# xandergos/terrain-diffusion

Measured on AMD Instinct MI355X. Metric: terrain megapixels/sec (decoded) at fixed steps, 30m model, higher is better.
Workload: dtype bf16; 1 GPU; BASELINE configs[2]: terrain-diffusion-30m base U-Net, 8x8 tile grid (stride 32, 288x288 latents) with overlap blending, 20 steps, 64 windows batched per solver step; edm_steps=20, parallelism=1 independent streams (one process per GPU, no data-path collective)

## Files before the change

### terrain_diffusion_amd/csrc/conv_fewcout.hip

```cpp
#include "conv_common.h"

namespace td {

template <typename T> __device__ __forceinline__ float fewcout_dot2(unsigned a, unsigned b, float c);
template <> __device__ __forceinline__ float fewcout_dot2<__bf16>(unsigned a, unsigned b, float c) {
    typedef __bf16 bx2 __attribute__((ext_vector_type(2)));
    return __builtin_amdgcn_fdot2_f32_bf16(__builtin_bit_cast(bx2, a), __builtin_bit_cast(bx2, b), c, false);
}
template <> __device__ __forceinline__ float fewcout_dot2<_Float16>(unsigned a, unsigned b, float c) {
    typedef _Float16 hx2 __attribute__((ext_vector_type(2)));
    return __builtin_amdgcn_fdot2(__builtin_bit_cast(hx2, a), __builtin_bit_cast(hx2, b), c, false);
}

template <typename T, int CO>
__global__ __launch_bounds__(256) void conv_fewcout_kernel(const ConvParams p) {
    constexpr int TW = 16, TH = 16, PW = 18, NPATCH = PW * PW, PITCH = 144, CHUNK = 64;
    constexpr int W_BASE = NPATCH * PITCH;
    extern __shared__ __attribute__((aligned(16))) unsigned char smem[];
    const int tid = threadIdx.x;
    unsigned b = blockIdx.x;
    const int txi = (int)(b % (unsigned)p.tiles_x); b /= (unsigned)p.tiles_x;
    const int tyi = (int)(b % (unsigned)p.tiles_y); const int n0 = (int)(b / (unsigned)p.tiles_y);
    const int y0 = tyi * TH, x0 = txi * TW;
    const ConvSeg& sg = p.seg[0];
// ... 34 lines not shown
                const u32x4 xv = *(const u32x4*)(xp + q * 16);
#pragma unroll
                for (int c = 0; c < CO; ++c) {
                    const u32x4 wv = *(const u32x4*)(smem + W_BASE + ((tap * CO + c) * 8 + q) * 16);
                    float a = acc[c][q >> 2];
#pragma unroll
                    for (int i = 0; i < 4; ++i) a = fewcout_dot2<T>(xv[i], wv[i], a);
                    acc[c][q >> 2] = a;
                }
            }
        }
    }
    const int y = y0 + ly, x = x0 + lx;
    if (y < H && x < W) {
        if (p.epi == EPI_DPM_STEP) {
            f32x4 v = {0.f, 0.f, 0.f, 0.f};
#pragma unroll
            for (int c = 0; c < CO; ++c) v[c] = acc[c][0] + acc[c][1];
            (void)epilogue4<T>(p, n0, y, x, 0, v, 0.f, v);
            return;
        }
        float* o = (float*)p.out + (size_t)((n0 * H + y) * W + x) * p.out_cstride;
#pragma unroll
        for (int c = 0; c < CO; ++c) if (c < p.Cout) o[c] = acc[c][0] + acc[c][1];
    }
}

template <typename T, int CO>
static hipError_t launch_fewcout_cfg(const ConvParams& p, hipStream_t st) {
    constexpr size_t LDS = (size_t)18 * 18 * 144 + (size_t)9 * CO * 128;
    const long long grid = (long long)p.tiles_x * p.tiles_y * p.N;
    if (grid <= 0 || grid >= ((long long)1 << 31)) return hipErrorInvalidValue;
    hipLaunchKernelGGL((conv_fewcout_kernel<T, CO>), dim3((unsigned)grid), dim3(256), LDS, st, p);
    return hipGetLastError();
}

hipError_t launch_conv_fewcout(const ConvParams& p, int dtype, hipStream_t st) {
    if (p.nseg != 1 || p.seg[0].taps != 9 || p.seg[0].xform != 0 || p.seg[0].resample != 0 || p.seg[0].Hs != p.H || p.seg[0].Ws != p.W || (p.seg[0].C & 63) || p.seg[0].C < 64)
        return hipErrorInvalidValue;
    if (p.epi == EPI_DPM_STEP && (!p.dpm_x || !p.dpm_m1 || !p.dpm_xin || p.dpm_xin_cstride < p.Cout || (p.dpm_k.order == 3 && !p.dpm_m2))) return hipErrorInvalidValue;
    if ((p.epi != EPI_PLAIN && p.epi != EPI_DPM_STEP) || !p.out_f32 || p.ksplit != 1 || p.res || p.out2 || p.out_sumsq || p.clip > 0.f || p.Cout < 1 || p.Cout > 4 || p.out_cstride < p.Cout)
        return hipErrorInvalidValue;
    if (p.tiles_x != (p.W + 15) / 16 || p.tiles_y != (p.H + 15) / 16) return hipErrorInvalidValue;
    const int co = p.Cout <= 1 ? 1 : p.Cout <= 2 ? 2 : 4;
    if (dtype == 2) return co == 1 ? launch_fewcout_cfg<_Float16, 1>(p, st) : co == 2 ? launch_fewcout_cfg<_Float16, 2>(p, st) : launch_fewcout_cfg<_Float16, 4>(p, st);
    return co == 1 ? launch_fewcout_cfg<__bf16, 1>(p, st) : co == 2 ? launch_fewcout_cfg<__bf16, 2>(p, st) : launch_fewcout_cfg<__bf16, 4>(p, st);
}

}
```

### terrain_diffusion_amd/csrc/conv_glds_wide.hip

```cpp
#include "conv_common.h"

namespace td {

#ifdef TD_TRACE
#define TDW_T(v) unsigned long long v = __builtin_amdgcn_s_memtime(); asm volatile("s_waitcnt lgkmcnt(0)" ::: "memory")
#define TDW_TACC(acc, a, b) acc += (b) - (a)
#else
#define TDW_T(v)
#define TDW_TACC(acc, a, b)
#endif

template <typename T, int BN, bool TAIL, bool PERS>
__global__ __launch_bounds__(256, 2) void conv_glds_kernel_wide(const ConvParams p) {
    static_assert(!(TAIL && PERS), "the persistent tile loop serves pure 3x3 launches");
    typedef typename Half<T>::x8 hx8;
    constexpr int NTHR = 256, TH = 16, TW = 16, TPIX = 256;
    constexpr int PW = 18, NPATCH = 18 * 18;
    constexpr int WM = 64, MT = 2, NT = BN / 32;
    constexpr int CHUNK = 64, HALF = 32, PER16 = 8;
    constexpr int WNT = PERS ? 128 : NTHR, PNT = PERS ? 128 : NTHR;
    constexpr int A_ITERS = (NPATCH * 4 + PNT - 1) / PNT;
    constexpr int A_FULL = NPATCH * 4 / PNT, A_REM = NPATCH * 4 - A_FULL * PNT;
    constexpr int NBI = (BN * 64 + WNT * 16 - 1) / (WNT * 16), PSTR = WNT * 16;
    constexpr int H_BYTES = BN * 64, RING = 4;
    constexpr bool HAS_DUMP = (BN * 64) % (WNT * 16) != 0;
    constexpr int DUMP_BASE = RING * H_BYTES;
    constexpr int PITCH = 80;
    constexpr int A_BASE = DUMP_BASE + (HAS_DUMP ? 2048 : 0), A_BYTES = NPATCH * PITCH;
    constexpr int RN_BASE = A_BASE + 2 * A_BYTES, RN_BYTES = (NPATCH * 4 + 15) / 16 * 16;
// ... 126 lines not shown
#define TDW_STORE_A(BUF, RNP) TDW_STORE_R(BUF, RNP, 0, A_ITERS)
#define TDW_STORE_R(BUF, RNP, I0, I1)                                                                  \
    {                                                                                                  \
        _Pragma("unroll") for (int it_ = (I0); it_ < (I1); ++it_) {                                    \
            if (it_ < A_FULL || pt < A_REM) {                                                          \
                u32x4 v_ = aoff[it_] >= 0 ? av[it_] : u32x4{0u, 0u, 0u, 0u};                           \
                if (seg_xform != 0 && aoff[it_] >= 0) {                                \
                    float s_ = seg_scale;                                                              \
                    if (seg_xform == 2) s_ *= (RNP)[(pt >> 2) + it_ * (PNT / 4)];                      \
                    v_ = xform_piece<T>(v_, s_);                                                       \
                }                                                                                      \
                *(u32x4*)(smem + st_base + ((BUF) * A_BYTES + it_ * (PNT / 4) * PITCH)) = v_;          \
            }                                                                                          \
        }                                                                                              \
    }
    const bool r_want = !TAIL && k_epi == EPI_RESIDUAL && k_hres;
    bool r_pref = false;
    const T* r_ptr[MT];
#define TDW_R_ADDR()                                                                                                  \
    {                                                                                                                 \
        TDW_FRESH()                                                                                                   \
        const int rHs_ = KA(res_Hs), rWs_ = KA(res_Ws), rrs_ = KA(res_resample), rcs_ = KA(res_cstride);              \
        _Pragma("unroll") for (int i_ = 0; i_ < MT; ++i_) {                                                           \
            int img_, ty_, tx_;                                                                                       \
            frag_pixel<TW, TPIX>(wm * WM + i_ * 32, l31, img_, ty_, tx_);                                             \
            const int y_ = y0 + ty_, x_ = x0 + tx_;                                                                   \
            const int sp_ = (n0 < k_N && y_ < k_H && x_ < k_W) ? src_pixel(n0, y_, x_, rHs_, rWs_, rrs_) : 0;         \
            r_ptr[i_] = (const T*)KA(res) + (sp_ * rcs_ + co0 + 8 * lh);                                              \
        }                                                                                                             \
    }
#define TDW_R_UNIT(Q) (*(const u32x4*)(r_ptr[(Q) / NU] + ((co0 + (((Q) % NU) >> 1) * 32 < k_Cout) ? (((Q) % NU) >> 1) * 32 + ((Q) & 1) * 16 : 0)))
// ... 62 lines not shown
#define TDW_FRAG_READ(WF, XF, SLOT, KS, BUF, TOFF)                                                           \
    {                                                                                                        \
        _Pragma("unroll") for (int j_ = 0; j_ < NT; ++j_) WF[j_] = *(const u32x4*)(smem + (wbase[KS] + (SLOT)) + j_ * 2048);    \
        _Pragma("unroll") for (int i_ = 0; i_ < MT; ++i_) XF[i_] = *(const u32x4*)(smem + xbase[i_] + ((BUF) * A_BYTES + (TOFF) + (KS) * 32)); \
    }
#define TDW_FRAG_MFMA(WF, XF)                                                                                \
    {                                                                                                        \
        _Pragma("unroll") for (int i_ = 0; i_ < MT; ++i_)                                                    \
            _Pragma("unroll") for (int j_ = 0; j_ < NT; ++j_)                                                \
                acc[i_][j_] = Half<T>::mfma32(__builtin_bit_cast(hx8, WF[j_]), __builtin_bit_cast(hx8, XF[i_]), acc[i_][j_]); \
    }
#define TDW_HS(S)                                                                                            \
    {                                                                                                        \
        TDW_T(tA_);                                                                                          \
         \
        if ((S) == 1 || (S) == 2 || (((S) == 10 || (S) == 11) && nxt)) asm volatile("s_waitcnt vmcnt(%0)" ::"n"(A_ITERS + NBI) : "memory"); \
        else if ((S) >= 16 && !nxt) { if (r_now) asm volatile("s_waitcnt vmcnt(%0)" ::"n"(A_ITERS) : "memory"); else asm volatile("s_waitcnt vmcnt(0)" ::: "memory"); } \
        else asm volatile("s_waitcnt vmcnt(%0)" ::"n"(NBI) : "memory");                                      \
        if ((S) == 6 || (S) == 15) asm volatile("s_waitcnt lgkmcnt(0)" ::: "memory");    \
        TDW_T(tM_); TDW_TACC(tr_stage, tA_, tM_);    \
        __builtin_amdgcn_s_barrier();                                                                        \
        asm volatile("" ::: "memory");                                                                       \
        TDW_T(tB_); TDW_TACC(tr_wait, tA_, tB_);                                                             \
        if ((S) == 3 || ((S) == 12 && nxt)) TDW_PIN_A()    \
        if ((S) + 3 < 18 || nxt) TDW_DMA((S) + 3);    \
        if ((S) == 0) TDW_LOAD_A(chunk, 1);                                                                  \
        if ((S) == 9 && nxt) { if (newseg) TDW_SEG_BEGIN(seg + 1); TDW_LOAD_A(newseg ? 0 : chunk + 1, 0); }  \
        if ((S) == 15 && r_now) TDW_LOAD_R()                                                                 \
        if ((S) == 5) TDW_STORE_A(1, s_rn);                                                                        \
        if ((S) == 14 && nxt) TDW_STORE_A(0, s_rn);                                                                \
        TDW_FRAG_MFMA(wfA_, xfA_);                                                                           \
        if ((S) < 17 || nxt) TDW_FRAG_READ(wfA_, xfA_, rslot, 0, (((S) + 1) / 9) & 1, TDW_TOFF(((S) + 1) % 9)); \
        TDW_FRAG_MFMA(wfB_, xfB_);                                                                           \
        if ((S) < 17 || nxt) { TDW_FRAG_READ(wfB_, xfB_, rslot, 1, (((S) + 1) / 9) & 1, TDW_TOFF(((S) + 1) % 9)); TDW_SLOT_NEXT(rslot) } \
        __builtin_amdgcn_sched_group_barrier(0x008, MT * NT, 0);                                             \
        __builtin_amdgcn_sched_group_barrier(0x100, NT + MT, 0);                                             \
        __builtin_amdgcn_sched_group_barrier(0x008, MT * NT, 0);                                             \
        __builtin_amdgcn_sched_group_barrier(0x100, NT + MT, 0);                                             \
    }
#define TDW_B0 4
#define TDW_B1 8
#define TDW_HSP(S)                                                                                           \
    {                                                                                                        \
        if (w_role) {                                                                                        \
            if ((S) >= 16 && !nxt) asm volatile("s_waitcnt vmcnt(0)" ::: "memory");                          \
            else if (((S) == 10 || (S) == 11) && nxt) asm volatile("s_waitcnt vmcnt(%0)" ::"n"(NBI + 1) : "memory"); \
            else asm volatile("s_waitcnt vmcnt(%0)" ::"n"(NBI) : "memory");                                  \
        } else {                                                                                             \
            if ((S) == 5 || ((S) == 14 && nxt)) asm volatile("s_waitcnt vmcnt(%0)" ::"n"(A_ITERS - TDW_B0) : "memory"); \
// ... 52 lines not shown
        asm volatile("" ::: "memory");
        TDW_FRAG_READ(wfA_, xfA_, rslot, 0, 0, TDW_TOFF(0));
        TDW_FRAG_READ(wfB_, xfB_, rslot, 1, 0, TDW_TOFF(0));
        TDW_SLOT_NEXT(rslot)
    }
    const bool no_tail = n3 == p.kgroups;
#ifdef TD_TRACE
    unsigned long long tr_loop = 0;
#endif
    for (;;) {
    const bool has_next = PERS && vb + vstep < k_grid;
    if (n3 > 0) {
        for (int u = 0; u < n3; ++u) {
            const bool last = u + 1 == n3;
            const bool wrap = PERS && last && has_next;
            const bool nxt = !last || wrap;
            const bool newseg = !last && chunk + 1 == seg_nchunks;
            const bool r_now = r_want && last && no_tail;
            if constexpr (PERS) {
                TDW_HSP(0); TDW_HSP(1); TDW_HSP(2); TDW_HSP(3); TDW_HSP(4); TDW_HSP(5); TDW_HSP(6); TDW_HSP(7); TDW_HSP(8);
                TDW_HSP(9); TDW_HSP(10); TDW_HSP(11); TDW_HSP(12); TDW_HSP(13); TDW_HSP(14); TDW_HSP(15); TDW_HSP(16); TDW_HSP(17);
            } else {
                TDW_HS(0); TDW_HS(1); TDW_HS(2); TDW_HS(3); TDW_HS(4); TDW_HS(5); TDW_HS(6); TDW_HS(7); TDW_HS(8);
                TDW_HS(9); TDW_HS(10); TDW_HS(11); TDW_HS(12); TDW_HS(13); TDW_HS(14); TDW_HS(15); TDW_HS(16); TDW_HS(17);
            }
            if (wrap) { seg = 0; chunk = 0; } else if (newseg) { ++seg; chunk = 0; } else ++chunk;
        }
    }
    if constexpr (TAIL) {
    if (n3 < p.kgroups && p.dma1x1) {
        constexpr int STAGE = TPIX * 64, NSTG = 3;
        static_assert(NSTG * STAGE <= 2 * A_BYTES, "stage buffers over the two halo patches");
        int pseg = n3 > 0 ? seg + 1 : 0, pchunk = 0, phf = 0, pn = 1;
        const T* psrc = nullptr;
        unsigned poff[4];
#define TDW_P_BEGIN()                                                                                                 \
// ... 225 lines not shown
#ifdef TD_TRACE
    TDW_T(tr_eissue);
    asm volatile("s_waitcnt vmcnt(0)" ::: "memory");
    TDW_T(tr_end);
    if (lane == 0) {
        unsigned long long* tb = (unsigned long long*)p.partial + ((size_t)blockIdx.x * 4 + wave) * 16;
        tb[0] = tr_pro - tr_start; tb[1] = tr_loop - tr_pro; tb[2] = tr_end - tr_loop; tb[3] = tr_wait; tb[4] = tr_stage; tb[5] = tr_start; tb[6] = tr_end;
        tb[8] = tr_rt0; tb[9] = ((unsigned long long)__builtin_amdgcn_s_getreg((31 << 11) | 4) << 8) | __builtin_amdgcn_s_getreg((3 << 11) | 20);
        tb[10] = __builtin_amdgcn_s_memrealtime();
        tb[7] = tb[10] - tr_rt0; tb[11] = tr_end - tr_eissue;
    }
#endif
#undef TDW_R_ADDR
#undef TDW_R_UNIT
#undef TDW_LOAD_R
}

template <typename T, int BN, bool TAIL, bool PERS>
static hipError_t launch_glds_wide_cfg2(const ConvParams& p, hipStream_t st) {
    constexpr int NPATCH = 18 * 18;
    constexpr size_t RING_BYTES = 4 * (size_t)(BN * 64) + ((BN * 64) % 4096 ? 2048 : 0);
    constexpr size_t LDS = RING_BYTES + 2 * (size_t)NPATCH * 80 + (PERS ? 2 : 1) * ((size_t)(NPATCH * 4 + 15) / 16 * 16 + (PERS ? (size_t)512 : (size_t)BN * 4));
    static_assert(2 * LDS <= 160 * 1024, "two workgroups per CU");
    if (p.ksplit != 1 || p.W < 16 || p.CoutPad % BN || p.nseg < 1 || p.nseg > 3) return hipErrorInvalidValue;
    if (p.out_f32 || (p.Cout & 7) || p.epi == EPI_DPM_STEP) return hipErrorInvalidValue;
    bool seen1 = false;
    for (int s = 0; s < p.nseg; ++s) { if (p.seg[s].taps == 9 && seen1) return hipErrorInvalidValue; if (p.seg[s].taps != 9) seen1 = true; }
    ConvParams pd = p;
    for (int s = p.nseg; s < 3; ++s) { pd.seg[s].C = 0; pd.seg[s].taps = 0; }
    pd.dma1x1 = 1;
    for (int s = 0; s < p.nseg; ++s) if (p.seg[s].taps != 9 && p.seg[s].xform != 0) pd.dma1x1 = 0;
    const int mtiles = p.tiles_x * p.tiles_y * p.img_groups, grid = p.n_ntiles * mtiles;
    if (grid <= 0 || (long long)grid * std::max(mtiles, p.n_ntiles) >= ((long long)1 << 32)) return hipErrorInvalidValue;
    pd.sb_d0 = mtiles; pd.sb_m0 = td_magic(mtiles); pd.sb_d1 = p.n_ntiles; pd.sb_m1 = td_magic(p.n_ntiles); pd.sb_m2 = td_magic(p.tiles_x); pd.sb_m3 = td_magic(p.tiles_y);
    pd.sb_grid = grid; pd.sb_grid8 = (grid & 7) == 0 ? (unsigned)grid >> 3 : 0u;
    int launch_grid = grid;
    if (PERS) {
        if (p.persist <= 0 || p.persist > grid || (p.H & 15) || (p.W & 15) || p.Cout != p.CoutPad || p.kgroups < 1) return hipErrorInvalidValue;
        if (pd.sb_grid8 && (p.persist & 7)) return hipErrorInvalidValue;
        launch_grid = p.persist;
    }
    auto kern = conv_glds_kernel_wide<T, BN, TAIL, PERS>;
    static bool attr_set[64] = {};
    int dev_ = 0; (void)hipGetDevice(&dev_);
    if (dev_ < 0 || dev_ >= 64 || !attr_set[dev_]) {
        hipError_t e = hipFuncSetAttribute((const void*)kern, hipFuncAttributeMaxDynamicSharedMemorySize, (int)LDS);
        if (e != hipSuccess) return e;
        if (dev_ >= 0 && dev_ < 64) attr_set[dev_] = true;
    }
    hipLaunchKernelGGL(kern, dim3(launch_grid), dim3(256), LDS, st, pd);
    return hipGetLastError();
}

inline int conv_wide_persist_grid(long long tiles, int slots) {
    if (tiles < 2LL * slots) return 0;
    const long long rounds = (tiles + slots - 1) / slots;
    long long g = (tiles + rounds - 1) / rounds;
    if ((tiles & 7) == 0) g = (g + 7) & ~7LL;
    return (int)std::min<long long>(g, tiles);
}

template <typename T, int BN>
static hipError_t launch_glds_wide_cfg(const ConvParams& p, hipStream_t st) {
    bool tail = false;
    for (int s = 0; s < p.nseg; ++s) if (p.seg[s].taps != 9) tail = true;
    if (p.persist > 0) {
        if constexpr (BN == 64) return tail ? hipErrorInvalidValue : launch_glds_wide_cfg2<T, BN, false, true>(p, st);
        else return hipErrorInvalidValue;
    }
    return tail ? launch_glds_wide_cfg2<T, BN, true, false>(p, st) : launch_glds_wide_cfg2<T, BN, false, false>(p, st);
}

hipError_t launch_conv_glds_wide(const ConvParams& p, int dtype, int bn, hipStream_t st) {
    if (dtype == 2) {
        if (bn == 96) return launch_glds_wide_cfg<_Float16, 96>(p, st);
        if (bn == 64) return launch_glds_wide_cfg<_Float16, 64>(p, st);
        return hipErrorInvalidValue;
    }
    if (bn == 96) return launch_glds_wide_cfg<__bf16, 96>(p, st);
    if (bn == 64) return launch_glds_wide_cfg<__bf16, 64>(p, st);
    return hipErrorInvalidValue;
}

}
```

### terrain_diffusion_amd/csrc/engine.hip

```cpp
#include <hip/hip_runtime.h>
#include <math.h>
#include <stdio.h>
#include <string.h>

#include <map>
#include <memory>
#include <string>
#include <vector>
#include <unordered_map>

#include "../../include/td_engine.h"
#include "td_device.h"

#include "conv_igemm.hip"
#include "conv_glds.hip"
#include "conv_glds_wide.hip"
#include "conv_sb.hip"
#include "conv_s16.hip"
#include "conv_fewcout.hip"
#include "small_kernels.hip"
#include "compose_kernels.hip"
#include "attn_mfma.hip"

using namespace td;
// ... 589 lines not shown
static int new_buf(Plan& pl, size_t bytes, void** out) {
    Buf b(new DevBuf());
    HIP_TRY(b->alloc(bytes, true));
    *out = b->p;
    pl.bytes += b->bytes;
    pl.bufs.push_back(std::move(b));
    return TD_OK;
}

struct SegSpec { const Tensor* t; int C; int taps; int resample; int xform; float scale; };

static int build_plan(td_unet* u, int N, int H, int W, Plan** out, int lane = 0) {
    static const char* const kPlanOptions[] = {"batch_invariant", "glds", "splitk", "producer_act", "glds_min_wgs", "glds_variant", "glds_bn",
                                               "glds_splitk", "glds_splitk_max", "glds_splitk_min_groups", "splitk_target_wgs",
                                               "bn128_min_wgs", "attn_mfma", "glds_splitk_from_groups", "glds_bn64", "glds_small_max_groups", "glds_round_aware", "walk_alternate", "glds_tiny", "glds_dma1x1", "splitk_weighted",
                                               "sb", "sb_target_wgs", "sb_mt", "sb_nt", "sb_order", "sb_max_glds_wgs", "sb_splitk", "sb_splitk_wgs", "sb_splitk_max", "s16", "s16_min_wgs", "sb_m4", "glds_wide", "glds_wide_min_wgs", "glds_wide_tail", "glds_wide_persist", "fewcout"};
    std::string key = std::to_string(N) + "_" + std::to_string(H) + "_" + std::to_string(W);
    for (const char* o : kPlanOptions) key += "_" + std::to_string((long long)u->eng->option(o, -7));
    if (lane) key += "_lane" + std::to_string(lane);
    auto it = u->plans.find(key);
    if (it != u->plans.end()) { it->second->last_use = ++u->use_clock; *out = it->second.get(); return TD_OK; }
    if (N < 1 || N > 1023 || H > 1023 || W > 1023) return fail(TD_ERR_ARG, "batch/size out of range");
    const int down = 1 << (u->cfg.n_levels - 1);
    if (H % down || W % down) return fail(TD_ERR_ARG, "H and W must be divisible by 2^(levels-1)");
    {
        const size_t budget = (size_t)u->eng->option("plan_cache_mb", 65536) << 20;
        const size_t max_plans = (size_t)u->eng->option("plan_cache_max", 12);
        size_t total = 0;
        for (auto& kv : u->plans) total += kv.second->bytes;
        while (!u->plans.empty() && (total > budget || u->plans.size() >= max_plans)) {
            auto victim = u->plans.begin();
// ... 36 lines not shown
        memset(&p, 0, sizeof p);
        p.nseg = (int)segs.size();
        int kgroups = 0;
        for (int i = 0; i < p.nseg; ++i) {
            const SegSpec& s = segs[i];
            ConvSeg& d = p.seg[i];
            d.src = s.t->ptr; d.C = (s.C + chunk - 1) / chunk * chunk; d.cstride = s.t->cstride; d.Hs = s.t->H; d.Ws = s.t->W;
            if ((size_t)N * d.Hs * d.Ws * (size_t)d.cstride >= ((size_t)1 << 31))
                return fail(TD_ERR_ARG, "batch too large for 32-bit activation addressing (N*H*W*C >= 2^31 elements in " + label + "): split the batch");
            d.taps = s.taps; d.resample = s.resample; d.xform = s.xform; d.scale = s.scale;
            if (s.xform == 2) {
                if (!s.t->sumsq) return fail(TD_ERR_STATE, "pixel-norm source without sumsq: " + label);
                d.sumsq = s.t->sumsq; d.nparts = s.t->nparts; d.inv_c = 1.f / (float)s.t->C;
            }
            kgroups += d.C / chunk;
            op.k_alg += (double)cw.segs[i].c_real * s.taps;
            if (cw.segs[i].c_pad != d.C || cw.segs[i].taps != d.taps) return fail(TD_ERR_STATE, "segment/weight mismatch: " + label);
        }
        p.wpack = cw.packed->p;
        p.N = N; p.H = h; p.W = w; p.Cout = cw.cout; p.CoutPad = cw.cout_pad; p.kgroups = kgroups;
        op.narrow = w < 16;
        {
            const int TW2 = op.narrow ? 8 : 16;
            const bool c128 = cw.cout_pad % 128 == 0, c96 = cw.cout_pad % 96 == 0;
            auto tiles = [&](int TH, int NIMG) { return (int64_t)((w + TW2 - 1) / TW2) * ((h + TH - 1) / TH) * ((N + NIMG - 1) / NIMG); };
            const bool c64 = !op.narrow && u->eng->option("glds_bn64", 1) != 0;
            auto pick_bn = [&](int64_t mt) { return (c128 && (mt * (cw.cout_pad / 128) >= 512 || !c96)) ? 128 : (c96 ? 96 : (c64 ? 64 : 0)); };
            const int64_t mt_big = tiles(op.narrow ? 8 : 16, op.narrow ? 4 : 1), mt_small = tiles(8, op.narrow ? 2 : 1);
            int variant = 0, bn2 = pick_bn(mt_big);
            if (bn2 && mt_big * (cw.cout_pad / bn2) < 1024) { variant = 1; bn2 = pick_bn(mt_small); }
// ... 32 lines not shown
                {
                    const int64_t wmode = u->eng->option("glds_wide", 1);
                    const int bnw = cw.cout_pad % 96 == 0 ? 96 : (cw.cout_pad % 64 == 0 ? 64 : 0);
                    const int64_t tmode = u->eng->option("glds_wide_tail", 1);
                    bool pure3 = true;
                    for (const SegSpec& sg : segs) if (sg.taps != 9 && (sg.xform != 0 || tmode == 0 || (tmode == 1 && bnw != 64))) pure3 = false;
                    const int64_t wgs_w = bnw ? tiles(16, 1) * (cw.cout_pad / bnw) : 0;
                    if (wmode != 0 && !inv && fv < 0 && fbn == 0 && !op.narrow && p.ksplit == 1 && bnw && !out_f32 && (cw.cout & 7) == 0 && p.nseg <= 3 && (pure3 || wmode == 2) &&
                        (wmode == 2 || wgs_w >= u->eng->option("glds_wide_min_wgs", 384))) {
                        op.glds_variant = 3; op.bn = bnw;
                        p.tiles_x = (w + 15) / 16; p.tiles_y = (h + 15) / 16; p.img_groups = N; p.n_ntiles = cw.cout_pad / bnw;
                        bool tail3 = false;
                        for (const SegSpec& sg : segs) if (sg.taps != 9) tail3 = true;
                        if (u->eng->option("glds_wide_persist", 0) != 0 && bnw == 64 && !tail3 && (h & 15) == 0 && (w & 15) == 0 && cw.cout == cw.cout_pad)
                            p.persist = conv_wide_persist_grid((long long)p.tiles_x * p.tiles_y * N * p.n_ntiles, 2 * std::max(1, u->eng->n_cus));
                    }
                }
                if (op.flavor == 2 && sb_takes && op.glds_variant != 3) {
                    {
                        const int TWs = op.narrow ? 8 : 16;
                        auto th_of = [&](int mt) { return op.narrow ? (mt == 2 ? 8 : 4) : (mt == 4 ? 8 : mt == 2 ? 4 : 2); };
                        auto sb_wgs = [&](int mt, int nt) { return (int64_t)((w + TWs - 1) / TWs) * ((h + th_of(mt) - 1) / th_of(mt)) * N * (cw.cout_pad / (32 * nt)); };
                        const int64_t target = u->eng->option("sb_target_wgs", 160);
                        int mt = 1, nt = 1, ks = 1;
                        if (!op.narrow && u->eng->option("sb_m4", 0) != 0 && sb_wgs(2, 2) >= target && sb_wgs(4, 1) >= target) { mt = 4; nt = 1; }
                        else if (sb_wgs(2, 2) >= target) { mt = 2; nt = 2; } else if (sb_wgs(2, 1) >= target) { mt = 2; nt = 1; }
                        else if (use_splitk && u->eng->option("sb_splitk", 1) != 0 && sb_wgs(2, 1) * 2 <= u->eng->option("sb_splitk_wgs", 224)) {
                            mt = 2; nt = 1;
                            ks = (int)std::min<int64_t>(std::min<int64_t>(kgroups, u->eng->option("sb_splitk_max", 16)), (u->eng->option("sb_splitk_wgs", 224) + sb_wgs(2, 1) / 2) / sb_wgs(2, 1));
                        }
// ... 30 lines not shown
            }
        }
        if (op.flavor == 0) {
            const int TH = 8, TW = op.narrow ? 8 : 16, NIMG = op.narrow ? 2 : 1;
            p.tiles_x = (w + TW - 1) / TW; p.tiles_y = (h + TH - 1) / TH; p.img_groups = (N + NIMG - 1) / NIMG;
            const int64_t mt = (int64_t)p.tiles_x * p.tiles_y * p.img_groups;
            op.bn = 64;
            const bool inv0 = u->eng->option("batch_invariant", 0) != 0;
            if (cw.cout_pad % 128 == 0 && (inv0 || mt * (cw.cout_pad / 128) >= bn128_min)) op.bn = 128;
            else if (cw.cout_pad % 96 == 0 && (inv0 || mt * (cw.cout_pad / 96) >= bn128_min)) op.bn = 96;
            p.n_ntiles = cw.cout_pad / op.bn;
            const int64_t base = mt * p.n_ntiles;
            p.ksplit = 1;
            if (use_splitk && !u->eng->option("batch_invariant", 0) && base < splitk_target / 2 && kgroups > 1) p.ksplit = (int)std::min<int64_t>(kgroups, (splitk_target + base - 1) / base);
        }
        if (u->eng->option("fewcout", 1) != 0 && (u->dt == 1 || u->dt == 2) && out_f32 && epi == EPI_PLAIN && cw.cout <= 4 && segs.size() == 1 && segs[0].taps == 9 &&
            segs[0].xform == 0 && p.seg[0].resample == 0 && p.seg[0].Hs == h && p.seg[0].Ws == w && !res && clip <= 0.f && (int64_t)h * w >= 128 * 128 && w >= 16) {
            op.flavor = 6; op.bn = 64; op.glds_variant = 0; op.narrow = false;
            p.tiles_x = (w + 15) / 16; p.tiles_y = (h + 15) / 16; p.img_groups = N; p.n_ntiles = 1; p.ksplit = 1; p.persist = 0;
        }
        if (p.ksplit > 64) p.ksplit = 64;
        if (!conv_set_kbounds(p, u->eng->option("splitk_weighted", 1) != 0, chunk)) return fail(TD_ERR_UNSUPPORTED, "split-K bounds: " + label);
        p.epi = epi; p.out_f32 = out_f32 ? 1 : 0; p.clip = clip; p.zeros = u->eng->zeros;
        const int out_parts = p.ksplit > 1 ? (cw.cout_pad + 255) / 256 : op.flavor == 5 ? cw.cout_pad / 16 : (op.flavor >= 2 ? cw.cout_pad / 32 : p.n_ntiles * 2);
        if (out_f32) {
            outT->C = cw.cout; outT->cstride = 8; outT->H = h; outT->W = w; outT->sumsq = nullptr;
            if ((rc = new_buf(pl, (size_t)N * h * w * 8 * 4, &outT->ptr))) return rc;
        } else if ((rc = new_tensor(cw.cout, h, w, want_sumsq, out_parts, outT))) return rc;
        p.out = outT->ptr; p.out_cstride = outT->cstride; p.out_sumsq = outT->sumsq;
        if ((size_t)N * h * w * (size_t)std::max(outT->cstride, cw.cout_pad) >= ((size_t)1 << 31))
            return fail(TD_ERR_ARG, "batch too large for 32-bit activation addressing (output of " + label + "): split the batch");
        op.cvec_off = cvec_off; p.cvec_stride = u->c_total;
        if (res) {
            p.res = res->ptr; p.res_cstride = res->cstride; p.res_Hs = res->H; p.res_Ws = res->W; p.res_resample = res_resample;
// ... 237 lines not shown
        }
        mark();
        hipError_t e = op.flavor == 6 ? launch_conv_fewcout(p, u->dt, st)
                       : op.flavor == 5 ? launch_conv_s16(p, u->dt, op.narrow, st)
                       : op.flavor == 4 ? launch_conv_sb(p, u->dt, op.narrow, op.sb_mt, op.sb_nt, st)
                       : op.flavor == 2 ? (op.glds_variant == 3 ? launch_conv_glds_wide(p, u->dt, op.bn, st) : launch_conv_glds(p, u->dt, op.narrow, op.bn, op.glds_variant, st))
                       : launch_conv(p, u->dt, op.narrow, op.bn, 0, st);
        mark(); if (prof) { ev_kind.push_back(0); char tag[160]; double gf_ = op.k_alg * 2.0 * p.N * p.H * p.W * p.Cout * 1e-9;
            double mb_ = 0.0; const double es_ = (double)u->esize();
            for (int si_ = 0; si_ < p.nseg; ++si_) mb_ += (double)p.N * p.seg[si_].Hs * p.seg[si_].Ws * p.seg[si_].C * es_ + (double)p.seg[si_].C / 64.0 * p.seg[si_].taps * p.CoutPad * 128.0 * (es_ / 2.0);
            if (p.res) mb_ += (double)p.N * p.res_Hs * p.res_Ws * p.Cout * es_;
            const double o1_ = (double)p.N * p.H * p.W * p.Cout * (p.out_f32 ? 4.0 : es_);
            const double mbs_ = (mb_ + o1_) * 1e-6;
            mb_ += o1_ * (p.out2 ? 2.0 : 1.0);
            mb_ *= 1e-6;
            snprintf(tag, sizeof tag, " [%dx%d k%d f%d%s bn%d wg%d ks%d gf%.2f mb%.2f mbs%.2f]", p.H, p.W, p.kgroups, op.flavor, op.flavor == 5 ? "c16" : op.flavor == 4 ? (op.sb_mt == 4 ? "m4n1" : op.sb_mt == 2 ? (op.sb_nt == 2 ? "m2n2" : "m2n1") : (op.sb_nt == 2 ? "m1n2" : "m1n1")) : op.flavor == 2 ? (op.glds_variant == 3 ? (p.persist > 0 ? "wp" : "w") : op.glds_variant == 2 ? "t" : op.glds_variant ? "s" : "b") : "", op.bn, p.n_ntiles * p.tiles_x * p.tiles_y * p.img_groups, p.ksplit, gf_, mb_, mbs_); ev_label.push_back(op.label + tag);
            ev_flop.push_back(op.flavor == 2 ? 2.0 * p.N * p.H * p.W * (double)p.Cout * op.k_alg : 0.0); }
        if (e != hipSuccess) return fail(TD_ERR_HIP, "conv launch " + op.label + ": " + hipGetErrorString(e));
    }
    return TD_OK;
}

static inline dim3 grid1(size_t n, int b = 256) { return dim3((unsigned)((n + b - 1) / b)); }

extern "C" {

const char* td_last_error(void) { return g_err.c_str(); }
int td_version(void) { return 1; }
#ifndef TD_CSRC_SHA
#define TD_CSRC_SHA "unstamped"
#endif
// ... 34 lines not shown
    DevGuard dg_(e->device); HIP_TRY(hipStreamSynchronize(e->stream)); e->deferred.clear(); e->ring.reset(); return TD_OK; }
void* td_engine_stream(td_engine* e) { return (void*)e->stream; }
int td_engine_set_stream(td_engine* e, void* hip_stream) {
    if (!e) return fail(TD_ERR_ARG, "null engine");
    DevGuard dg_(e->device);
    HIP_TRY(hipStreamSynchronize(e->stream));
    e->deferred.clear();
    e->ring.reset();
    e->stream = hip_stream ? (hipStream_t)hip_stream : e->own_stream;
    return TD_OK;
}
static const char* const kKnownOptions[] = {
    "async", "batch_invariant", "fuse_solver", "graph", "lower_order_final", "profile", "solver_order", "dual_stream", "dual_stream_min_batch", "sampler_stop_after",
    "plan_cache_mb", "plan_cache_max",
    "attn_mfma", "bn128_min_wgs", "glds", "glds_bn", "glds_bn64", "glds_dma1x1", "glds_min_wgs", "glds_round_aware", "glds_small_max_groups",
    "glds_splitk", "glds_splitk_from_groups", "glds_splitk_max", "glds_splitk_min_groups", "glds_tiny", "glds_variant", "glds_wide", "glds_wide_min_wgs", "glds_wide_tail", "glds_wide_persist", "fewcout",
    "producer_act", "s16", "s16_min_wgs", "sb", "sb_m4", "sb_max_glds_wgs", "sb_mt", "sb_nt", "sb_order", "sb_splitk", "sb_splitk_max", "sb_splitk_wgs", "sb_target_wgs", "splitk",
    "splitk_target_wgs", "splitk_weighted", "walk_alternate"};
int td_engine_set_option(td_engine* e, const char* key, int64_t value) {
    if (!e || !key) return fail(TD_ERR_ARG, "null");
    bool known = false;
    for (const char* k : kKnownOptions) known = known || strcmp(k, key) == 0;
    if (!known) return fail(TD_ERR_ARG, std::string("unknown engine option \"") + key + "\" (include/td_engine.h lists the options)");
    e->opt[key] = value;
    return TD_OK;
}

int td_engine_profile_read(td_engine* e, double* conv_ms, int64_t* conv_launches, double* other_ms, int64_t* other_launches, int reset) {
    if (conv_ms) *conv_ms = e->prof_conv_ms;
    if (conv_launches) *conv_launches = e->prof_conv_launches;
    if (other_ms) *other_ms = e->prof_other_ms;
// ... 729 lines not shown
```

### terrain_diffusion_amd/csrc/td_device.h

```cpp
#pragma once
#include <hip/hip_runtime.h>
#include <stdint.h>

namespace td {

struct ConvSeg {
    const void* src;
    const float* sumsq;
    int C;
    int cstride;
    int Hs, Ws;
    int taps;
    int resample;
    int xform;
    int nparts;
    float scale;
    float inv_c;
};

struct SchedCoef {
    float c_skip, c_out;
    float a, b0, inv_r0;
    float inv_r1, f01, inv_r01, c1, c2;
    float c_in_next;
// ... 50 lines not shown
    float out2_scale;
    const void* zeros;
    float* dpm_x;
    float* dpm_m1;
    float* dpm_m2;
    void* dpm_xin;
    int dpm_xin_cstride;
    SchedCoef dpm_k;
    int reverse;
    int dma1x1;
    int persist;
    const void* wpack_sb;
    int sb_n3;
    int sb_order;
    unsigned sb_d0, sb_m0, sb_d1, sb_m1, sb_m2, sb_m3, sb_grid8, sb_grid;
};

inline bool conv_set_kbounds(ConvParams& p, bool weighted, int chunk = 64) {
    if (p.ksplit < 1 || p.ksplit > 64 || p.kgroups > 255 || p.ksplit > p.kgroups) return false;
    int wt[256], n = 0, total = 0; bool mixed = false;
    for (int s = 0; s < p.nseg; ++s)
        for (int c = 0; c < p.seg[s].C / chunk && n < 256; ++c) { wt[n] = p.seg[s].taps; mixed = mixed || wt[n] != wt[0]; total += wt[n]; ++n; }
    if (n != p.kgroups) return false;
    p.kb[0] = 0; p.kb[p.ksplit] = (unsigned char)n;
    int g = 0, acc = 0;
    for (int s = 1; s < p.ksplit; ++s) {
        int b;
        if (!(weighted && mixed)) b = (int)((long)s * n / p.ksplit);
        else {
            const long target = (long)s * total;
// ... 15 lines not shown
```

Before: 21.36 MP/s.

## Add half-K wide conv variant for ≤32-channel inputs; extend fewcout kernel to 8 outputs

Result: no change. 21.46 MP/s (median of 4 runs) (+0.4%).

```diff
diff --git a/terrain_diffusion_amd/csrc/conv_fewcout.hip b/terrain_diffusion_amd/csrc/conv_fewcout.hip
--- a/terrain_diffusion_amd/csrc/conv_fewcout.hip
+++ b/terrain_diffusion_amd/csrc/conv_fewcout.hip
@@ -72,10 +72,13 @@
     const int y = y0 + ly, x = x0 + lx;
     if (y < H && x < W) {
         if (p.epi == EPI_DPM_STEP) {
-            f32x4 v = {0.f, 0.f, 0.f, 0.f};
 #pragma unroll
-            for (int c = 0; c < CO; ++c) v[c] = acc[c][0] + acc[c][1];
-            (void)epilogue4<T>(p, n0, y, x, 0, v, 0.f, v);
+            for (int c0 = 0; c0 < CO; c0 += 4) {
+                f32x4 v = {0.f, 0.f, 0.f, 0.f};
+#pragma unroll
+                for (int c = c0; c < CO && c < c0 + 4; ++c) v[c - c0] = acc[c][0] + acc[c][1];
+                (void)epilogue4<T>(p, n0, y, x, c0, v, 0.f, v);
+            }
             return;
         }
         float* o = (float*)p.out + (size_t)((n0 * H + y) * W + x) * p.out_cstride;
@@ -93,16 +96,28 @@
     return hipGetLastError();
 }
 
+template <typename T>
+static hipError_t launch_fewcout_co(const ConvParams& p, hipStream_t st) {
+    switch (p.Cout) {
+        case 1: return launch_fewcout_cfg<T, 1>(p, st);
+        case 2: return launch_fewcout_cfg<T, 2>(p, st);
+        case 3: case 4: return launch_fewcout_cfg<T, 4>(p, st);
+        case 5: return launch_fewcout_cfg<T, 5>(p, st);
+        case 6: return launch_fewcout_cfg<T, 6>(p, st);
+        case 7: return launch_fewcout_cfg<T, 7>(p, st);
+        default: return launch_fewcout_cfg<T, 8>(p, st);
+    }
+}
+
 hipError_t launch_conv_fewcout(const ConvParams& p, int dtype, hipStream_t st) {
     if (p.nseg != 1 || p.seg[0].taps != 9 || p.seg[0].xform != 0 || p.seg[0].resample != 0 || p.seg[0].Hs != p.H || p.seg[0].Ws != p.W || (p.seg[0].C & 63) || p.seg[0].C < 64)
         return hipErrorInvalidValue;
     if (p.epi == EPI_DPM_STEP && (!p.dpm_x || !p.dpm_m1 || !p.dpm_xin || p.dpm_xin_cstride < p.Cout || (p.dpm_k.order == 3 && !p.dpm_m2))) return hipErrorInvalidValue;
-    if ((p.epi != EPI_PLAIN && p.epi != EPI_DPM_STEP) || !p.out_f32 || p.ksplit != 1 || p.res || p.out2 || p.out_sumsq || p.clip > 0.f || p.Cout < 1 || p.Cout > 4 || p.out_cstride < p.Cout)
+    if ((p.epi != EPI_PLAIN && p.epi != EPI_DPM_STEP) || !p.out_f32 || p.ksplit != 1 || p.res || p.out2 || p.out_sumsq || p.clip > 0.f || p.Cout < 1 || p.Cout > 8 || p.out_cstride < p.Cout)
         return hipErrorInvalidValue;
     if (p.tiles_x != (p.W + 15) / 16 || p.tiles_y != (p.H + 15) / 16) return hipErrorInvalidValue;
-    const int co = p.Cout <= 1 ? 1 : p.Cout <= 2 ? 2 : 4;
-    if (dtype == 2) return co == 1 ? launch_fewcout_cfg<_Float16, 1>(p, st) : co == 2 ? launch_fewcout_cfg<_Float16, 2>(p, st) : launch_fewcout_cfg<_Float16, 4>(p, st);
-    return co == 1 ? launch_fewcout_cfg<__bf16, 1>(p, st) : co == 2 ? launch_fewcout_cfg<__bf16, 2>(p, st) : launch_fewcout_cfg<__bf16, 4>(p, st);
+    if (dtype == 2) return launch_fewcout_co<_Float16>(p, st);
+    return launch_fewcout_co<__bf16>(p, st);
 }
 
 }
diff --git a/terrain_diffusion_amd/csrc/conv_glds_wide.hip b/terrain_diffusion_amd/csrc/conv_glds_wide.hip
--- a/terrain_diffusion_amd/csrc/conv_glds_wide.hip
+++ b/terrain_diffusion_amd/csrc/conv_glds_wide.hip
@@ -1,3 +1,4 @@
+#ifndef TDW_BODY
 #include "conv_common.h"
 
 namespace td {
@@ -10,9 +11,10 @@
 #define TDW_TACC(acc, a, b)
 #endif
 
-template <typename T, int BN, bool TAIL, bool PERS>
-__global__ __launch_bounds__(256, 2) void conv_glds_kernel_wide(const ConvParams p) {
+#else
     static_assert(!(TAIL && PERS), "the persistent tile loop serves pure 3x3 launches");
+    static_assert(!HSKIP || (!TAIL && !PERS), "the half-unit form serves one-unit 3x3 launches");
+    constexpr int LAST_S = HSKIP ? 8 : 17;
     typedef typename Half<T>::x8 hx8;
     constexpr int NTHR = 256, TH = 16, TW = 16, TPIX = 256;
     constexpr int PW = 18, NPATCH = 18 * 18;
@@ -169,7 +171,7 @@
             }                                                                                          \
         }                                                                                              \
     }
-    const bool r_want = !TAIL && k_epi == EPI_RESIDUAL && k_hres;
+    const bool r_want = !TAIL && !HSKIP && k_epi == EPI_RESIDUAL && k_hres;
     bool r_pref = false;
     const T* r_ptr[MT];
 #define TDW_R_ADDR()                                                                                                  \
@@ -262,25 +264,25 @@
     {                                                                                                        \
         TDW_T(tA_);                                                                                          \
          \
-        if ((S) == 1 || (S) == 2 || (((S) == 10 || (S) == 11) && nxt)) asm volatile("s_waitcnt vmcnt(%0)" ::"n"(A_ITERS + NBI) : "memory"); \
-        else if ((S) >= 16 && !nxt) { if (r_now) asm volatile("s_waitcnt vmcnt(%0)" ::"n"(A_ITERS) : "memory"); else asm volatile("s_waitcnt vmcnt(0)" ::: "memory"); } \
+        if (!HSKIP && ((S) == 1 || (S) == 2 || (((S) == 10 || (S) == 11) && nxt))) asm volatile("s_waitcnt vmcnt(%0)" ::"n"(A_ITERS + NBI) : "memory"); \
+        else if ((S) >= LAST_S - 1 && !nxt) { if (r_now) asm volatile("s_waitcnt vmcnt(%0)" ::"n"(A_ITERS) : "memory"); else asm volatile("s_waitcnt vmcnt(0)" ::: "memory"); } \
         else asm volatile("s_waitcnt vmcnt(%0)" ::"n"(NBI) : "memory");                                      \
-        if ((S) == 6 || (S) == 15) asm volatile("s_waitcnt lgkmcnt(0)" ::: "memory");    \
+        if (!HSKIP && ((S) == 6 || (S) == 15)) asm volatile("s_waitcnt lgkmcnt(0)" ::: "memory");    \
         TDW_T(tM_); TDW_TACC(tr_stage, tA_, tM_);    \
         __builtin_amdgcn_s_barrier();                                                                        \
         asm volatile("" ::: "memory");                                                                       \
         TDW_T(tB_); TDW_TACC(tr_wait, tA_, tB_);                                                             \
-        if ((S) == 3 || ((S) == 12 && nxt)) TDW_PIN_A()    \
-        if ((S) + 3 < 18 || nxt) TDW_DMA((S) + 3);    \
-        if ((S) == 0) TDW_LOAD_A(chunk, 1);                                                                  \
+        if (!HSKIP && ((S) == 3 || ((S) == 12 && nxt))) TDW_PIN_A()    \
+        if ((S) + 3 <= LAST_S || nxt) TDW_DMA((S) + 3);    \
+        if (!HSKIP && (S) == 0) TDW_LOAD_A(chunk, 1);                                                        \
         if ((S) == 9 && nxt) { if (newseg) TDW_SEG_BEGIN(seg + 1); TDW_LOAD_A(newseg ? 0 : chunk + 1, 0); }  \
         if ((S) == 15 && r_now) TDW_LOAD_R()                                                                 \
-        if ((S) == 5) TDW_STORE_A(1, s_rn);                                                                        \
+        if (!HSKIP && (S) == 5) TDW_STORE_A(1, s_rn);                                                              \
         if ((S) == 14 && nxt) TDW_STORE_A(0, s_rn);                                                                \
         TDW_FRAG_MFMA(wfA_, xfA_);                                                                           \
-        if ((S) < 17 || nxt) TDW_FRAG_READ(wfA_, xfA_, rslot, 0, (((S) + 1) / 9) & 1, TDW_TOFF(((S) + 1) % 9)); \
+        if ((S) < LAST_S || nxt) TDW_FRAG_READ(wfA_, xfA_, rslot, 0, (((S) + 1) / 9) & 1, TDW_TOFF(((S) + 1) % 9)); \
         TDW_FRAG_MFMA(wfB_, xfB_);                                                                           \
-        if ((S) < 17 || nxt) { TDW_FRAG_READ(wfB_, xfB_, rslot, 1, (((S) + 1) / 9) & 1, TDW_TOFF(((S) + 1) % 9)); TDW_SLOT_NEXT(rslot) } \
+        if ((S) < LAST_S || nxt) { TDW_FRAG_READ(wfB_, xfB_, rslot, 1, (((S) + 1) / 9) & 1, TDW_TOFF(((S) + 1) % 9)); TDW_SLOT_NEXT(rslot) } \
         __builtin_amdgcn_sched_group_barrier(0x008, MT * NT, 0);                                             \
         __builtin_amdgcn_sched_group_barrier(0x100, NT + MT, 0);                                             \
         __builtin_amdgcn_sched_group_barrier(0x008, MT * NT, 0);                                             \
@@ -363,12 +365,14 @@
         for (int u = 0; u < n3; ++u) {
             const bool last = u + 1 == n3;
             const bool wrap = PERS && last && has_next;
-            const bool nxt = !last || wrap;
+            const bool nxt = !HSKIP && (!last || wrap);
             const bool newseg = !last && chunk + 1 == seg_nchunks;
             const bool r_now = r_want && last && no_tail;
             if constexpr (PERS) {
                 TDW_HSP(0); TDW_HSP(1); TDW_HSP(2); TDW_HSP(3); TDW_HSP(4); TDW_HSP(5); TDW_HSP(6); TDW_HSP(7); TDW_HSP(8);
                 TDW_HSP(9); TDW_HSP(10); TDW_HSP(11); TDW_HSP(12); TDW_HSP(13); TDW_HSP(14); TDW_HSP(15); TDW_HSP(16); TDW_HSP(17);
+            } else if constexpr (HSKIP) {
+                TDW_HS(0); TDW_HS(1); TDW_HS(2); TDW_HS(3); TDW_HS(4); TDW_HS(5); TDW_HS(6); TDW_HS(7); TDW_HS(8);
             } else {
                 TDW_HS(0); TDW_HS(1); TDW_HS(2); TDW_HS(3); TDW_HS(4); TDW_HS(5); TDW_HS(6); TDW_HS(7); TDW_HS(8);
                 TDW_HS(9); TDW_HS(10); TDW_HS(11); TDW_HS(12); TDW_HS(13); TDW_HS(14); TDW_HS(15); TDW_HS(16); TDW_HS(17);
@@ -624,9 +628,23 @@
 #undef TDW_R_ADDR
 #undef TDW_R_UNIT
 #undef TDW_LOAD_R
+#endif
+#ifndef TDW_BODY
+#define TDW_BODY
+template <typename T, int BN, bool TAIL, bool PERS>
+__global__ __launch_bounds__(256, 2) void conv_glds_kernel_wide(const ConvParams p) {
+    constexpr bool HSKIP = false;
+#include "conv_glds_wide.hip"
 }
 
-template <typename T, int BN, bool TAIL, bool PERS>
+template <typename T, int BN>
+__global__ __launch_bounds__(256, 2) void conv_glds_kernel_wide_half(const ConvParams p) {
+    constexpr bool TAIL = false, PERS = false, HSKIP = true;
+#include "conv_glds_wide.hip"
+}
+#undef TDW_BODY
+
+template <typename T, int BN, bool TAIL, bool PERS, bool HSKIP = false>
 static hipError_t launch_glds_wide_cfg2(const ConvParams& p, hipStream_t st) {
     constexpr int NPATCH = 18 * 18;
     constexpr size_t RING_BYTES = 4 * (size_t)(BN * 64) + ((BN * 64) % 4096 ? 2048 : 0);
@@ -650,7 +668,10 @@
         if (pd.sb_grid8 && (p.persist & 7)) return hipErrorInvalidValue;
         launch_grid = p.persist;
     }
-    auto kern = conv_glds_kernel_wide<T, BN, TAIL, PERS>;
+    if (HSKIP != (p.half_skip != 0)) return hipErrorInvalidValue;
+    if (HSKIP && (p.nseg != 1 || p.kgroups != 1 || p.seg[0].taps != 9 || p.seg[0].C != 64 || p.seg_creal[0] < 1 || p.seg_creal[0] > 32)) return hipErrorInvalidValue;
+    void (*kern)(const ConvParams);
+    if constexpr (HSKIP) kern = conv_glds_kernel_wide_half<T, BN>; else kern = conv_glds_kernel_wide<T, BN, TAIL, PERS>;
     static bool attr_set[64] = {};
     int dev_ = 0; (void)hipGetDevice(&dev_);
     if (dev_ < 0 || dev_ >= 64 || !attr_set[dev_]) {
@@ -678,6 +699,7 @@
         if constexpr (BN == 64) return tail ? hipErrorInvalidValue : launch_glds_wide_cfg2<T, BN, false, true>(p, st);
         else return hipErrorInvalidValue;
     }
+    if (p.half_skip) return tail ? hipErrorInvalidValue : launch_glds_wide_cfg2<T, BN, false, false, true>(p, st);
     return tail ? launch_glds_wide_cfg2<T, BN, true, false>(p, st) : launch_glds_wide_cfg2<T, BN, false, false>(p, st);
 }
 
@@ -693,3 +715,4 @@
 }
 
 }
+#endif
diff --git a/terrain_diffusion_amd/csrc/engine.hip b/terrain_diffusion_amd/csrc/engine.hip
--- a/terrain_diffusion_amd/csrc/engine.hip
+++ b/terrain_diffusion_amd/csrc/engine.hip
@@ -627,7 +627,7 @@
     static const char* const kPlanOptions[] = {"batch_invariant", "glds", "splitk", "producer_act", "glds_min_wgs", "glds_variant", "glds_bn",
                                                "glds_splitk", "glds_splitk_max", "glds_splitk_min_groups", "splitk_target_wgs",
                                                "bn128_min_wgs", "attn_mfma", "glds_splitk_from_groups", "glds_bn64", "glds_small_max_groups", "glds_round_aware", "walk_alternate", "glds_tiny", "glds_dma1x1", "splitk_weighted",
-                                               "sb", "sb_target_wgs", "sb_mt", "sb_nt", "sb_order", "sb_max_glds_wgs", "sb_splitk", "sb_splitk_wgs", "sb_splitk_max", "s16", "s16_min_wgs", "sb_m4", "glds_wide", "glds_wide_min_wgs", "glds_wide_tail", "glds_wide_persist", "fewcout"};
+                                               "sb", "sb_target_wgs", "sb_mt", "sb_nt", "sb_order", "sb_max_glds_wgs", "sb_splitk", "sb_splitk_wgs", "sb_splitk_max", "s16", "s16_min_wgs", "sb_m4", "glds_wide", "glds_wide_min_wgs", "glds_wide_tail", "glds_wide_persist", "fewcout", "glds_half_skip"};
     std::string key = std::to_string(N) + "_" + std::to_string(H) + "_" + std::to_string(W);
     for (const char* o : kPlanOptions) key += "_" + std::to_string((long long)u->eng->option(o, -7));
     if (lane) key += "_lane" + std::to_string(lane);
@@ -694,6 +694,7 @@
                 d.sumsq = s.t->sumsq; d.nparts = s.t->nparts; d.inv_c = 1.f / (float)s.t->C;
             }
             kgroups += d.C / chunk;
+            p.seg_creal[i] = cw.segs[i].c_real;
             op.k_alg += (double)cw.segs[i].c_real * s.taps;
             if (cw.segs[i].c_pad != d.C || cw.segs[i].taps != d.taps) return fail(TD_ERR_STATE, "segment/weight mismatch: " + label);
         }
@@ -756,6 +757,9 @@
                         for (const SegSpec& sg : segs) if (sg.taps != 9) tail3 = true;
                         if (u->eng->option("glds_wide_persist", 0) != 0 && bnw == 64 && !tail3 && (h & 15) == 0 && (w & 15) == 0 && cw.cout == cw.cout_pad)
                             p.persist = conv_wide_persist_grid((long long)p.tiles_x * p.tiles_y * N * p.n_ntiles, 2 * std::max(1, u->eng->n_cus));
+                        if (u->eng->option("glds_half_skip", 1) != 0 && p.persist == 0 && p.nseg == 1 && segs[0].taps == 9 && kgroups == 1 && chunk == 64 &&
+                            cw.segs[0].c_real >= 1 && cw.segs[0].c_real <= 32)
+                            p.half_skip = 1;
                     }
                 }
                 if (op.flavor == 2 && sb_takes && op.glds_variant != 3) {
@@ -816,10 +820,14 @@
             p.ksplit = 1;
             if (use_splitk && !u->eng->option("batch_invariant", 0) && base < splitk_target / 2 && kgroups > 1) p.ksplit = (int)std::min<int64_t>(kgroups, (splitk_target + base - 1) / base);
         }
-        if (u->eng->option("fewcout", 1) != 0 && (u->dt == 1 || u->dt == 2) && out_f32 && epi == EPI_PLAIN && cw.cout <= 4 && segs.size() == 1 && segs[0].taps == 9 &&
-            segs[0].xform == 0 && p.seg[0].resample == 0 && p.seg[0].Hs == h && p.seg[0].Ws == w && !res && clip <= 0.f && (int64_t)h * w >= 128 * 128 && w >= 16) {
-            op.flavor = 6; op.bn = 64; op.glds_variant = 0; op.narrow = false;
-            p.tiles_x = (w + 15) / 16; p.tiles_y = (h + 15) / 16; p.img_groups = N; p.n_ntiles = 1; p.ksplit = 1; p.persist = 0;
+        {
+            const int64_t ftiles = (int64_t)((w + 15) / 16) * ((h + 15) / 16) * N;
+            const bool big_map = (int64_t)h * w >= 128 * 128, big_batch = u->eng->option("batch_invariant", 0) == 0 && ftiles >= 512;
+            if (u->eng->option("fewcout", 1) != 0 && (u->dt == 1 || u->dt == 2) && out_f32 && epi == EPI_PLAIN && cw.cout <= 8 && segs.size() == 1 && segs[0].taps == 9 &&
+                segs[0].xform == 0 && p.seg[0].resample == 0 && p.seg[0].Hs == h && p.seg[0].Ws == w && !res && clip <= 0.f && (big_map || big_batch) && w >= 16) {
+                op.flavor = 6; op.bn = 64; op.glds_variant = 0; op.narrow = false;
+                p.tiles_x = (w + 15) / 16; p.tiles_y = (h + 15) / 16; p.img_groups = N; p.n_ntiles = 1; p.ksplit = 1; p.persist = 0;
+            }
         }
         if (p.ksplit > 64) p.ksplit = 64;
         if (!conv_set_kbounds(p, u->eng->option("splitk_weighted", 1) != 0, chunk)) return fail(TD_ERR_UNSUPPORTED, "split-K bounds: " + label);
@@ -1087,7 +1095,7 @@
             const double mbs_ = (mb_ + o1_) * 1e-6;
             mb_ += o1_ * (p.out2 ? 2.0 : 1.0);
             mb_ *= 1e-6;
-            snprintf(tag, sizeof tag, " [%dx%d k%d f%d%s bn%d wg%d ks%d gf%.2f mb%.2f mbs%.2f]", p.H, p.W, p.kgroups, op.flavor, op.flavor == 5 ? "c16" : op.flavor == 4 ? (op.sb_mt == 4 ? "m4n1" : op.sb_mt == 2 ? (op.sb_nt == 2 ? "m2n2" : "m2n1") : (op.sb_nt == 2 ? "m1n2" : "m1n1")) : op.flavor == 2 ? (op.glds_variant == 3 ? (p.persist > 0 ? "wp" : "w") : op.glds_variant == 2 ? "t" : op.glds_variant ? "s" : "b") : "", op.bn, p.n_ntiles * p.tiles_x * p.tiles_y * p.img_groups, p.ksplit, gf_, mb_, mbs_); ev_label.push_back(op.label + tag);
+            snprintf(tag, sizeof tag, " [%dx%d k%d f%d%s bn%d wg%d ks%d gf%.2f mb%.2f mbs%.2f]", p.H, p.W, p.kgroups, op.flavor, op.flavor == 5 ? "c16" : op.flavor == 4 ? (op.sb_mt == 4 ? "m4n1" : op.sb_mt == 2 ? (op.sb_nt == 2 ? "m2n2" : "m2n1") : (op.sb_nt == 2 ? "m1n2" : "m1n1")) : op.flavor == 2 ? (op.glds_variant == 3 ? (p.persist > 0 ? "wp" : p.half_skip ? "wh" : "w") : op.glds_variant == 2 ? "t" : op.glds_variant ? "s" : "b") : "", op.bn, p.n_ntiles * p.tiles_x * p.tiles_y * p.img_groups, p.ksplit, gf_, mb_, mbs_); ev_label.push_back(op.label + tag);
             ev_flop.push_back(op.flavor == 2 ? 2.0 * p.N * p.H * p.W * (double)p.Cout * op.k_alg : 0.0); }
         if (e != hipSuccess) return fail(TD_ERR_HIP, "conv launch " + op.label + ": " + hipGetErrorString(e));
     }
@@ -1152,7 +1160,7 @@
     "async", "batch_invariant", "fuse_solver", "graph", "lower_order_final", "profile", "solver_order", "dual_stream", "dual_stream_min_batch", "sampler_stop_after",
     "plan_cache_mb", "plan_cache_max",
     "attn_mfma", "bn128_min_wgs", "glds", "glds_bn", "glds_bn64", "glds_dma1x1", "glds_min_wgs", "glds_round_aware", "glds_small_max_groups",
-    "glds_splitk", "glds_splitk_from_groups", "glds_splitk_max", "glds_splitk_min_groups", "glds_tiny", "glds_variant", "glds_wide", "glds_wide_min_wgs", "glds_wide_tail", "glds_wide_persist", "fewcout",
+    "glds_splitk", "glds_splitk_from_groups", "glds_splitk_max", "glds_splitk_min_groups", "glds_tiny", "glds_variant", "glds_wide", "glds_wide_min_wgs", "glds_wide_tail", "glds_wide_persist", "glds_half_skip", "fewcout",
     "producer_act", "s16", "s16_min_wgs", "sb", "sb_m4", "sb_max_glds_wgs", "sb_mt", "sb_nt", "sb_order", "sb_splitk", "sb_splitk_max", "sb_splitk_wgs", "sb_target_wgs", "splitk",
     "splitk_target_wgs", "splitk_weighted", "walk_alternate"};
 int td_engine_set_option(td_engine* e, const char* key, int64_t value) {
diff --git a/terrain_diffusion_amd/csrc/td_device.h b/terrain_diffusion_amd/csrc/td_device.h
--- a/terrain_diffusion_amd/csrc/td_device.h
+++ b/terrain_diffusion_amd/csrc/td_device.h
@@ -88,6 +88,8 @@
     int sb_n3;
     int sb_order;
     unsigned sb_d0, sb_m0, sb_d1, sb_m1, sb_m2, sb_m3, sb_grid8, sb_grid;
+    int seg_creal[3];
+    int half_skip;
 };
 
 inline bool conv_set_kbounds(ConvParams& p, bool weighted, int chunk = 64) {
```
